# agnusmaximus/Word2Bits

Hardware: AMD Instinct MI355X
Metric: training words/sec at dim=800 bitlevel=1 neg=24 (higher is better)
Workload: dtype f32

## Files before the change

include/word2bits_hip.h:

```cpp
#ifndef WORD2BITS_HIP_H
#define WORD2BITS_HIP_H
#include <stdint.h>
#ifdef __cplusplus
extern "C" {
#endif

#define W2B_OK            0
#define W2B_EINVAL       -1
#define W2B_ENOGPU       -2
#define W2B_EHIP         -3
#define W2B_ENOMEM       -4
#define W2B_EUNSUPPORTED -5
#define W2B_ERCCL        -6
#define W2B_ESTATE       -7
#define W2B_EIO          -8

#define W2B_EXP_TABLE_SIZE 1000
#define W2B_MAX_EXP 6
#define W2B_MAX_SENTENCE_LENGTH 1000
#define W2B_UNIGRAM_TABLE_SIZE 100000000LL

typedef struct w2b_trainer w2b_trainer;

typedef struct w2b_config {
// ... 76 lines not shown
int w2b_export_packed(w2b_trainer *t, uint64_t *out);

int w2b_set_vocab_counts(w2b_trainer *t, const int64_t *cn, int64_t table_size);
int w2b_set_unigram_table(w2b_trainer *t, const int32_t *table, int64_t table_size);
int w2b_set_exp_table(w2b_trainer *t, const float *exp_table);

int w2b_set_corpus(w2b_trainer *t, const int32_t *ids, int64_t n_tokens);
int w2b_set_corpus_device(w2b_trainer *t, const void *ids_dev, int64_t n_tokens);
int w2b_set_corpus_slice(w2b_trainer *t, const int32_t *ids, int64_t n_tokens, int32_t more_follows);
int w2b_set_shards(w2b_trainer *t, const int64_t *starts, const int32_t *first_override );
int w2b_epoch_begin(w2b_trainer *t);
int w2b_train_step(w2b_trainer *t, int64_t max_positions);
int w2b_epoch_status(w2b_trainer *t, int32_t *finished, int64_t *word_count_actual, float *alpha,
                     double *loss_sum);

int w2b_epoch_poll(w2b_trainer *t, int32_t lag, int32_t *finished, int64_t *word_count_actual, float *alpha,
                   double *loss_sum);

int w2b_suggested_threads(w2b_trainer *t, int32_t *out);

int w2b_worker_kernel_info(w2b_trainer *t, int32_t *resident, int32_t *radius, int32_t *column_bytes,
                           int32_t *workgroups_per_cu, int32_t *hot_rows);
int w2b_worker_kernel_lean(w2b_trainer *t, int32_t *lean);

int w2b_train_tuples(w2b_trainer *t, int64_t n, const int32_t *center, const int32_t *ctx_off,
                     const int32_t *ctx, const int32_t *neg, float alpha, int32_t serial,
                     double *loss_out );
int w2b_train_tuples_device(w2b_trainer *t, int64_t n, const void *center_dev, const void *ctx_off_dev,
                            const void *ctx_dev, const void *neg_dev, float alpha, int32_t grid);

int w2b_synchronize(w2b_trainer *t);
int w2b_timing_enable(w2b_trainer *t, int32_t on);
int w2b_timing_read(w2b_trainer *t, double *kernel_ms, int64_t *launches);
int w2b_timing_launches(w2b_trainer *t, double *ms_out, int64_t capacity, int64_t *launches);

#define W2B_UNIQUE_ID_BYTES 128
int w2b_comm_unique_id(void *out128);
int w2b_comm_init(w2b_trainer *t, int32_t nranks, int32_t rank, const void *id128);
int w2b_comm_count(w2b_trainer *t, int32_t *nranks_out);
int w2b_sync_replicas(w2b_trainer *t, int32_t mode);
int64_t w2b_suggested_exchange_words(int64_t train_words_per_epoch, int32_t replicas);
int w2b_sync_stats(w2b_trainer *t, int64_t *exchanges, double *device_ms);

int w2b_exchange_init(w2b_trainer *t);
int w2b_exchange_begin(w2b_trainer *t, int64_t *n_chunks, int64_t *local_word_count );
int w2b_exchange_counts(w2b_trainer *t, void **buf_dev, int64_t *elems);
// ... 61 lines not shown
```

word2bits_amd/_lib.py:

```python
import ctypes as C
import os
import sys

_HERE = os.path.dirname(os.path.abspath(__file__))
LIB_PATH = os.environ.get("W2B_LIB", os.path.join(_HERE, "libword2bits_hip.so"))

W2B_OK, W2B_EINVAL, W2B_ENOGPU, W2B_EHIP, W2B_ENOMEM = 0, -1, -2, -3, -4
W2B_EUNSUPPORTED, W2B_ERCCL, W2B_ESTATE, W2B_EIO = -5, -6, -7, -8
ERROR_NAMES = {-1: "W2B_EINVAL", -2: "W2B_ENOGPU", -3: "W2B_EHIP", -4: "W2B_ENOMEM",
               -5: "W2B_EUNSUPPORTED", -6: "W2B_ERCCL", -7: "W2B_ESTATE", -8: "W2B_EIO"}


class W2bError(RuntimeError):
    def __init__(self, code, text):
        super().__init__("%s (%d): %s" % (ERROR_NAMES.get(code, "?"), code, text))
        self.code = code


class Config(C.Structure):
    _fields_ = [
        ("vocab_size", C.c_int64), ("train_words", C.c_int64), ("iter", C.c_int64),
        ("layer1_size", C.c_int32), ("window", C.c_int32), ("negative", C.c_int32),
        ("bitlevel", C.c_int32), ("num_threads", C.c_int32),
        ("alpha", C.c_float), ("sample", C.c_float), ("reg", C.c_float),
# ... 38 lines not shown
    "w2b_plan_rows": (C.c_int, [C.POINTER(Config), C.POINTER(Tuning), i64p, C.c_int32, C.c_int32, C.POINTER(RowPlan)]),
    "w2b_get_tuning": (C.c_int, [vp, C.POINTER(Tuning)]),
    "w2b_set_tuning": (C.c_int, [vp, C.POINTER(Tuning)]),
    "w2b_init_net": (C.c_int, [vp]),
    "w2b_set_model": (C.c_int, [vp, f32p, f32p]),
    "w2b_get_model": (C.c_int, [vp, f32p, f32p]),
    "w2b_model_device_ptrs": (C.c_int, [vp, C.POINTER(vp), C.POINTER(vp)]),
    "w2b_export_quantized": (C.c_int, [vp, f32p]),
    "w2b_export_packed": (C.c_int, [vp, u64p]),
    "w2b_set_vocab_counts": (C.c_int, [vp, i64p, C.c_int64]),
    "w2b_set_unigram_table": (C.c_int, [vp, i32p, C.c_int64]),
    "w2b_set_exp_table": (C.c_int, [vp, f32p]),
    "w2b_set_corpus": (C.c_int, [vp, i32p, C.c_int64]),
    "w2b_set_corpus_device": (C.c_int, [vp, vp, C.c_int64]),
    "w2b_set_corpus_slice": (C.c_int, [vp, i32p, C.c_int64, C.c_int32]),
    "w2b_set_shards": (C.c_int, [vp, i64p, i32p]),
    "w2b_epoch_begin": (C.c_int, [vp]),
    "w2b_train_step": (C.c_int, [vp, C.c_int64]),
    "w2b_epoch_status": (C.c_int, [vp, i32p, i64p, f32p, f64p]),
    "w2b_epoch_poll": (C.c_int, [vp, C.c_int32, i32p, i64p, f32p, f64p]),
    "w2b_suggested_threads": (C.c_int, [vp, i32p]),
    "w2b_worker_kernel_info": (C.c_int, [vp, i32p, i32p, i32p, i32p, i32p]),
    "w2b_worker_kernel_lean": (C.c_int, [vp, i32p]),
    "w2b_train_tuples": (C.c_int, [vp, C.c_int64, i32p, i32p, i32p, i32p, C.c_float, C.c_int32, f64p]),
    "w2b_train_tuples_device": (C.c_int, [vp, C.c_int64, vp, vp, vp, vp, C.c_float, C.c_int32]),
    "w2b_synchronize": (C.c_int, [vp]),
    "w2b_timing_enable": (C.c_int, [vp, C.c_int32]),
    "w2b_timing_read": (C.c_int, [vp, f64p, i64p]),
    "w2b_timing_launches": (C.c_int, [vp, f64p, C.c_int64, i64p]),
    "w2b_comm_unique_id": (C.c_int, [vp]),
    "w2b_comm_init": (C.c_int, [vp, C.c_int32, C.c_int32, vp]),
    "w2b_comm_count": (C.c_int, [vp, i32p]),
    "w2b_sync_replicas": (C.c_int, [vp, C.c_int32]),
    "w2b_suggested_exchange_words": (C.c_int64, [C.c_int64, C.c_int32]),
    "w2b_sync_stats": (C.c_int, [vp, i64p, f64p]),
    "w2b_exchange_init": (C.c_int, [vp]),
    "w2b_exchange_begin": (C.c_int, [vp, i64p, i64p]),
    "w2b_exchange_counts": (C.c_int, [vp, C.POINTER(vp), i64p]),
    "w2b_exchange_delta": (C.c_int, [vp, C.c_int64, C.POINTER(vp), i64p]),
    "w2b_exchange_apply": (C.c_int, [vp, C.c_int64, C.c_float]),
    "w2b_exchange_end": (C.c_int, [vp, C.c_int64]),
    "w2b_corpus_load": (C.c_int, [C.c_char_p, C.c_int32, C.POINTER(vp)]),
    "w2b_corpus_load_ex": (C.c_int, [C.c_char_p, C.c_int32, C.c_int32, C.POINTER(vp)]),
    "w2b_corpus_free": (None, [vp]),
    "w2b_corpus_vocab_size": (C.c_int64, [vp]),
    "w2b_corpus_train_words": (C.c_int64, [vp]),
# ... 143 lines not shown
```

word2bits_amd/csrc/w2b_device.hpp:

```cpp
#pragma once
#include "w2b_internal.h"
#include <type_traits>

#ifndef W2B_T
#define W2B_T 13
#endif
#ifndef W2B_T_LOSS
#define W2B_T_LOSS W2B_T
#endif
template <bool LOSS> struct TFor { static constexpr int value = LOSS ? W2B_T_LOSS : W2B_T; };
#ifndef W2B_CA
#define W2B_CA 8
#endif
#ifndef W2B_STASH
#define W2B_STASH 8
#endif
#ifndef W2B_MINWAVES
#define W2B_MINWAVES 4
#endif

namespace {

struct QParam { int bitlevel; int steps_i; float steps_f; };

// ... 143 lines not shown
  f32x4_t t;
  t.x = c.e[0]; t.y = c.e[1]; t.z = c.e[2]; t.w = c.e[3];
  *(W2B_LDS f32x4_t *)p = t;
}

#ifdef W2B_PHASE_TIMERS
#define W2B_TICK(k) do { if (timing_) { const unsigned long long n_ = __builtin_readcyclecounter(); \
    atomicAdd(&P.shared->dbg[k], n_ - tick_); tick_ = n_; } } while (0)
#define W2B_COUNT(k) do { if (timing_) atomicAdd(&P.shared->dbg[k], 1ull); } while (0)
#else
#define W2B_TICK(k) do { } while (0)
#define W2B_COUNT(k) do { } while (0)
#endif

struct WordLds {
  int *ctx;
  int *umult;
  int *tgt;
  int *prev;
  int *cend;
  float *red;
  float *stash;
  float *xprod;
};

__device__ __forceinline__ int round4(int x) { return (x + 3) & ~3; }

__device__ __forceinline__ WordLds carve_word_lds(int *base, int window, int negative, int vec) {
  const int maxc = round4(2 * window + 1), maxt = round4(negative + 1);
  WordLds L;
  L.stash = reinterpret_cast<float *>(base);
  base += W2B_STASH * blockDim.x * vec;
  L.red = reinterpret_cast<float *>(base);
  int *p = base + 2 * W2B_T * W2B_MAXW;
  L.ctx = p; p += maxc;
  L.umult = p; p += maxc;
  L.tgt = p; p += maxt;
  L.prev = p; p += maxt;
  L.cend = p; p += maxt;
  L.xprod = nullptr;
  return L;
}


template <int T, typename IP>
__device__ __forceinline__ int prep_lists(IP tgt, IP prev, IP cend, int nt, IP ctx, IP umult, int cw,
                                          int lane) {
  W2B_WAVE_SYNC();
  for (int i0 = 0; i0 < nt; i0 += 64) {
    const int i = i0 + lane;
    const int me = (i < nt) ? tgt[i] : -1;
    int pd = -1;
    for (int j = 0; j < min(nt, i0 + 64); j++) {
      const int tj = (j >= i0) ? __builtin_amdgcn_readlane(me, j - i0) : tgt[j];
      pd = (j < i && tj == me) ? j : pd;
    }
    if (i < nt) prev[i] = pd;
  }
  if (umult) {
    for (int i0 = 0; i0 < cw; i0 += 64) {
      const int i = i0 + lane;
      const int me = (i < cw) ? ctx[i] : -1;
      bool first = true;
// ... 181 lines not shown
                                             double &loss_acc, const XHot &X) {
  static_assert(!LEAN || (VEC == 4 && MM == 0 && ATOM == 0 && TB == 0 && QM <= 2), "lean form: see w2b_workers_lean");
  constexpr bool REG = !LEAN;
  constexpr bool ATOM_U = !(VEC == 4 && ATOM < 1), ATOM_V = !(VEC == 4 && ATOM < 2);
  constexpr bool THIRDS = LEAN && QM == 1;
  constexpr float third = 1.f / 3.f;
  const int tid = threadIdx.x, lane = tid & 63, wave = tid >> 6, nwaves = blockDim.x >> 6;
  const int dim = P.dim, col0 = tid * VEC;
  const bool active = col0 < dim;
  const float ar2 = REG ? (2.f * alpha) * P.reg : 0.f;
  constexpr int TC = TFor<LOSS>::value;

  Col<VEC> x[TC];
  int rows[TC];
  int start = 0, chunk = 0, end = L.cend[0];
  auto chunk_rows = [&]() {
    const int mine = L.tgt[min(start + lane, nt - 1)];
#pragma unroll
    for (int i = 0; i < TC; i++) rows[i] = __builtin_amdgcn_readlane(mine, i);
  };
  chunk_rows();
  const int nhu = (VEC == 4) ? X.nu : 0, nhv = (VEC == 4) ? X.nv : 0;
  [[maybe_unused]] const int rowb = dim * 4, lane_off = active ? col0 * 4 : (int)W2B_NO_LANE;
  [[maybe_unused]] __amdgpu_buffer_rsrc_t res_u, res_v, res_cu, res_cv;
  if constexpr (LEAN) {
    res_u = __builtin_amdgcn_make_buffer_rsrc((void *)P.u, 0, (int)P.tab_bytes, 0x27000);
    res_v = __builtin_amdgcn_make_buffer_rsrc((void *)P.v, 0, (int)P.tab_bytes, 0x27000);
    res_cu = __builtin_amdgcn_make_buffer_rsrc((void *)X.cu, 0, nhu * rowb, 0x27000);
    res_cv = __builtin_amdgcn_make_buffer_rsrc((void *)X.cv, 0, nhv * rowb, 0x27000);
  }
  auto ld_u = [&](int row) -> Col<VEC> {
    if constexpr (VEC == 4) { if ((unsigned)(row - 1) < (unsigned)nhu) return xhot_ld(X.cu, row - 1, nhu, dim, col0); }
    return load_col<VEC, MM, TB>(P.u, row, dim, col0, P.tab_bytes);
  };
  [[maybe_unused]] const int atomic_rank = ATOM_V ? P.atomic_rank : 0, atomic_rank_u = ATOM_U ? P.atomic_rank_u : 0;
  auto up_u = [&](int row, const Col<VEC> &val, const Col<VEC> &d) {
    if constexpr (VEC == 4) { if ((unsigned)(row - 1) < (unsigned)nhu) { xhot_st(X.cu, row - 1, nhu, dim, col0, val); return; } }
    if constexpr (ATOM_U) { if (row <= atomic_rank_u) { add_col<VEC, TB>(P.u, row, dim, col0, d, P.tab_bytes); return; } }
    store_col<VEC, MM, TB>(P.u, row, dim, col0, val, P.tab_bytes);
  };
  auto ld_v = [&](int row) -> Col<VEC> {
    if constexpr (VEC == 4) { if ((unsigned)(row - 1) < (unsigned)nhv) return xhot_ld(X.cv, row - 1, nhv, dim, col0); }
    return load_col<VEC, MM, TB>(P.v, row, dim, col0, P.tab_bytes);
  };
  auto up_v = [&](int row, const Col<VEC> &val, const Col<VEC> &d) {
    if constexpr (VEC == 4) { if ((unsigned)(row - 1) < (unsigned)nhv) { xhot_st(X.cv, row - 1, nhv, dim, col0, val); return; } }
// ... 10 lines not shown
      if (zero) {
#pragma unroll
        for (int e = 0; e < VEC; e++) x[i].e[e] = 0.f;
      }
      if constexpr (LEAN) { if (start + i < end) x[i] = lean_ld_v(rows[i]); }
      else if (active && start + i < end) x[i] = ld_v(rows[i]);
    }
  };
  load_targets(true);

  Col<VEC> avg;
  float regsq = 0.f;
  const bool reg_on = REG && P.reg != 0.f;
  float *fsave = reinterpret_cast<float *>(L.prev);
#pragma unroll
  for (int e = 0; e < VEC; e++) avg.e[e] = 0.f;
  for (int j0 = 0; j0 < cw; j0 += W2B_CA) {
    Col<VEC> r[W2B_CA];
    if constexpr (LEAN) {
      const int mine = L.ctx[min(j0 + lane, cw - 1)];
#pragma unroll
      for (int jj = 0; jj < W2B_CA; jj++)
        if (j0 + jj < cw) r[jj] = lean_ld_u(__builtin_amdgcn_readlane(mine, jj));
    } else {
#pragma unroll
      for (int jj = 0; jj < W2B_CA; jj++)
        if (active && j0 + jj < cw) r[jj] = ld_u(__builtin_amdgcn_readfirstlane(L.ctx[j0 + jj]));
    }
#pragma unroll
    for (int jj = 0; jj < W2B_CA; jj++)
      if ((LEAN || active) && j0 + jj < cw) {
        if (j0 + jj < W2B_STASH) {
#pragma unroll
          for (int e = 0; e < VEC; e++) L.stash[((j0 + jj) * blockDim.x + tid) * VEC + e] = r[jj].e[e];
        }
#pragma unroll
        for (int e = 0; e < VEC; e++) {
          const float q = quant<QM>(r[jj].e[e], qp);
          avg.e[e] += q;
          if (LOSS && reg_on) regsq += q * q;
        }
      }
  }
  {
    const float cwf = (float)cw;
#pragma unroll
    for (int e = 0; e < VEC; e++) avg.e[e] = active ? avg.e[e] / cwf : 0.f;
  }
  [[maybe_unused]] Col<VEC> avg3;
  if constexpr (THIRDS) {
#pragma unroll
    for (int e = 0; e < VEC; e++) avg3.e[e] = avg.e[e] * third;
  }

  Col<VEC> err;
#pragma unroll
  for (int e = 0; e < VEC; e++) err.e[e] = 0.f;
  int par = 0;
  for (;;) {
    const int n = end - start;
    float p[TC];
#pragma unroll
    for (int i = 0; i < TC; i++) {
      float t[VEC];
#pragma unroll
      for (int e = 0; e < VEC; e++) {
        if constexpr (THIRDS) t[e] = (x[i].e[e] < 0.f) ? -avg3.e[e] : avg3.e[e];
        else {
          const float q = quant<QM>(x[i].e[e], qp);
          t[e] = avg.e[e] * q;
        }
      }
      const float s = (VEC == 4) ? (t[0] + t[1 % VEC]) + (t[2 % VEC] + t[3 % VEC]) : ((VEC == 2) ? t[0] + t[1 % VEC] : t[0]);
      p[i] = active ? s : 0.f;
    }
    float *red = L.red + par * (TC * W2B_MAXW);
    if (MM == W2B_MM_EXACT) {
      float fchain = 0.f;
      for (int b0 = 0; b0 < dim; b0 += W2B_EXACT_COLS) {
        if (active && col0 >= b0 && col0 < b0 + W2B_EXACT_COLS) {
#pragma unroll
          for (int i = 0; i < TC; i++)
            if (i < n) {
#pragma unroll
              for (int e = 0; e < VEC; e++)
                L.xprod[i * (W2B_EXACT_COLS + 1) + (col0 - b0) + e] = avg.e[e] * quant<QM>(x[i].e[e], qp);
            }
        }
        __syncthreads();
        if (wave == 0 && lane < n) {
          const int cnt = min(W2B_EXACT_COLS, dim - b0);
          const float *src = L.xprod + lane * (W2B_EXACT_COLS + 1);
          for (int c = 0; c < cnt; c++) fchain += src[c];
        }
        __syncthreads();
      }
      if (wave == 0 && lane < n) {
        red[lane * W2B_MAXW] = fchain;
        for (int w = 1; w < nwaves; w++) red[lane * W2B_MAXW + w] = 0.f;
      }
    } else {
#pragma unroll
      for (int i = 0; i < TC; i++) p[i] = wave_sum(p[i]);
      if (lane == 0) {
#pragma unroll
        for (int i = 0; i < TC; i++)
          if (i < n) red[i * W2B_MAXW + wave] = p[i];
      }
    }
    __syncthreads();
    float gl = 0.f;
    if (lane < n) {
      float f = 0.f;
      for (int w = 0; w < nwaves; w++) f += red[lane * W2B_MAXW + w];
      gl = grad_scalar(f, start + lane == 0, alpha, P.exp_table);
      if (LOSS && wave == 0) fsave[start + lane] = f;
    }
#pragma unroll
    for (int i = 0; i < TC; i++) {
      if (i < n) {
        const float g = __int_as_float(__builtin_amdgcn_readlane(__float_as_int(gl), i));
        [[maybe_unused]] const float g3 = g * third;
        const bool by_add = (VEC == 4 && ATOM >= 2) && rows[i] <= atomic_rank && !((unsigned)(rows[i] - 1) < (unsigned)nhv);
        Col<VEC> dl;
        if constexpr (VEC == 4 && ATOM >= 2) {
#pragma unroll
          for (int e = 0; e < VEC; e++) dl.e[e] = 0.f;
        }
        if constexpr (LEAN) {
#pragma unroll
          for (int h = 0; h < 4; h += 2) {
            f32x2_t xv = {x[i].e[h], x[i].e[h + 1]};
            if (QM != 0) asm volatile("" : "+v"(xv));
            f32x2_t ge;
            if constexpr (THIRDS) { ge.x = (xv.x < 0.f) ? -g3 : g3; ge.y = (xv.y < 0.f) ? -g3 : g3; }
            else { ge.x = quant<QM>(xv.x, qp); ge.y = quant<QM>(xv.y, qp); ge = g * ge; }
            const f32x2_t ev = f32x2_t{err.e[h], err.e[h + 1]} + ge;
            err.e[h] = ev.x; err.e[h + 1] = ev.y;
// ... 21 lines not shown
        }
        if constexpr (VEC == 4 && ATOM >= 2) {
          if (by_add) add_col_contig<TB>(P.v, rows[i], dim, dl, P.tab_bytes);
        }
      }
    }
    start = end;
    if (start >= nt) break;
    end = L.cend[++chunk];
    par ^= 1;
    chunk_rows();
    load_targets(false);
  }

  for (int j0 = 0; j0 < cw; j0 += W2B_CA) {
    Col<VEC> r[W2B_CA];
    if constexpr (LEAN) {
      const int mine = L.ctx[min(j0 + lane, cw - 1)], mult = (j0 + lane < cw) ? L.umult[min(j0 + lane, cw - 1)] : 0;
      const int how_l = (j0 + lane < W2B_STASH && mine > P.fresh_rank_u) ? mult : -mult;
      if (j0 < W2B_STASH) {
        static_assert(W2B_STASH % W2B_CA == 0, "a sub-chunk lies inside the stash or beyond it");
        Col<4> rs[W2B_CA];
#pragma unroll
        for (int jj = 0; jj < W2B_CA; jj++) rs[jj] = lds_ld((const W2B_LDS float *)(L.stash + ((j0 + jj) * blockDim.x + tid) * VEC));
#pragma unroll
        for (int jj = 0; jj < W2B_CA; jj++) {
          const int how = __builtin_amdgcn_readlane(how_l, jj);
          for (int k = 0; k < how; k++) {
#pragma unroll
            for (int e = 0; e < VEC; e++) rs[jj].e[e] = rs[jj].e[e] + err.e[e];
          }
          lean_st(res_u, res_cu, nhu, rowb, __builtin_amdgcn_readlane(mine, jj), how > 0 ? lane_off : (int)W2B_NO_LANE, rs[jj]);
        }
      }
      if (__ballot(lane < W2B_CA && how_l < 0) != 0ull) {
#pragma unroll
        for (int jj = 0; jj < W2B_CA; jj++)
          if (__builtin_amdgcn_readlane(how_l, jj) < 0) r[jj] = lean_ld_u(__builtin_amdgcn_readlane(mine, jj));
        __builtin_amdgcn_s_waitcnt(0x0F70);
#pragma unroll
        for (int jj = 0; jj < W2B_CA; jj++) {
          const int how = __builtin_amdgcn_readlane(how_l, jj);
          if (how < 0) {
            for (int k = 0; k < -how; k++) {
#pragma unroll
              for (int e = 0; e < VEC; e++) r[jj].e[e] = r[jj].e[e] + err.e[e];
            }
// ... 358 lines not shown
```

word2bits_amd/csrc/w2b_internal.h:

```cpp
#pragma once
#include <hip/hip_runtime.h>
#include <stdint.h>

#define W2B_LCG_A 25214903917ULL
#define W2B_LCG_C 11ULL
#define W2B_MAX_SEN 1000
#define W2B_MAXW 16
#define W2B_NXCD 8
#define W2B_XHOT_MAX 128

struct W2bShared {
  float alpha;
  int pad0;
  unsigned long long word_count_actual;
  double loss_tuples;
  int workers_done;
  int corpus_overrun;
  unsigned long long wca_others;
  unsigned long long wca_at_sync;
  double loss_epoch;
  int launch_done, pad1;
  unsigned long long dbg[16];
};

// ... 25 lines not shown
  unsigned long long table_magic, window_magic;
  int dim, window, negative, bitlevel, num_threads;
  int total_threads;
  int mem_mode;
  float *entry;
  float *xhot;
  int xhot_u, xhot_v;
  int hot_period;
  int xhot_m;
  int uavg_rank;
  int win_refresh;
  float xhot_w;
  float *wide_scratch;
  int wide;
  int atomic_rank;
  int atomic_rank_u;
  int fresh_rank_u;
  int exact;
  int rc_rows;
  float *rc;
  int *rc_flags;
  int worker_base;
  float starting_alpha, sample, reg;
};

struct w2b_config;
struct w2b_tuning;
void w2b_shape_params(W2bParams &p, const w2b_config &cfg, const w2b_tuning &tune);

int w2b_block_threads(int dim, int *vec_out, int *wide_out = nullptr);
size_t w2b_lds_bytes(int dim, int window, int negative, bool worker_form, bool exact = false);
int w2b_tuple_max_grid(int num_cus);
hipError_t w2b_launch_tuples(const W2bParams &p, long long n, const int32_t *center,
                             const int32_t *ctx_off, const int32_t *ctx, const int32_t *neg,
                             float alpha, int grid, int num_cus, int per_cu_override, bool loss,
                             hipStream_t s);
hipError_t w2b_launch_workers(const W2bParams &p, long long max_positions, bool loss, hipStream_t s, int grid = 0,
                              bool force_generic = false);
bool w2b_workers_lean(const W2bParams &p, bool force_generic);
int w2b_resident_plan(int dim, int window, int negative);
bool w2b_resident_atomic_ok(const W2bParams &p, int radius);
long long w2b_resident_scratch_rows(int radius);
hipError_t w2b_launch_resident(const W2bParams &p, long long max_positions, int radius, bool loss, hipStream_t s,
                               bool debug = false);
bool w2b_groups_ok(const W2bParams &p);
size_t w2b_groups_lds_bytes(int dim, int window, int negative);
int w2b_groups_per_cu(const W2bParams &p, bool loss);
hipError_t w2b_launch_groups(const W2bParams &p, long long max_positions, bool loss, hipStream_t s);
hipError_t w2b_launch_refresher(const W2bParams &p, hipStream_t s);
#define W2B_RC_MAX 64
#define W2B_RC_BLOCKS 16
int w2b_workers_per_cu(const W2bParams &p, bool loss);
int w2b_resident_per_cu(const W2bParams &p, int radius, bool loss);
hipError_t w2b_launch_init_net(float *u, float *v, long long n_per_table, const float *lut,
                               hipStream_t s);
hipError_t w2b_launch_export(const float *u, const float *v, float *out, long long n, int bitlevel,
                             hipStream_t s);
hipError_t w2b_launch_export_packed(const float *u, const float *v, unsigned long long *out, long long rows, int dim,
                                    int bitlevel, hipStream_t s);
hipError_t w2b_launch_eval_normalize(float *M, long long words, long long size, long long ld, int bitlevel,
                                     int fused, float *len_scratch, hipStream_t s);
hipError_t w2b_launch_eval_queries(const float *M, long long ld, long long nq, const int *b1, const int *b2,
                                   const int *b3, float *Q, int variant, hipStream_t s);
hipError_t w2b_launch_eval_scores(const float *Q, const float *M, int nq, int words, int size, int ld, int fused,
                                  const int *b1, const int *b2, const int *b3, unsigned long long *best,
                                  int variant , hipStream_t s);
void w2b_eval_topk_layout(long long words, int k, bool mfma, int *nunits, int *cap);
hipError_t w2b_launch_eval_topk(const float *Q, const float *M, int nq, int words, int size, int ld, int fused,
                                const int *b1, const int *b2, const int *b3, int k, unsigned long long *bound,
                                unsigned long long *bkt, unsigned long long *keys, unsigned char *cnt,
                                unsigned long long *out, int variant, hipStream_t s);
hipError_t w2b_launch_bits_planes(const uint32_t *B, int nw, int dim, int nq, long long nqp, const int *b1, const int *b2,
                                  const int *b3, uint32_t *P, hipStream_t s);
void w2b_bits_layout(long long words, long long nq, int topk, int max_splits, int *splits, int *rows_per_split);
hipError_t w2b_launch_bits_top1(const uint32_t *B, int words, int dim, const uint32_t *P, long long nqp, int nq,
// ... 129 lines not shown
```

word2bits_amd/csrc/w2b_kernels_misc.hip:

```cpp
#include "w2b_device.hpp"

namespace {
__global__ void k_init_net(float *u, float *v, long long n, const float *__restrict__ lut) {
  const long long stride = (long long)gridDim.x * blockDim.x;
  for (long long i = (long long)blockIdx.x * blockDim.x + threadIdx.x; i < n; i += stride) {
    v[i] = lut[i & 65535];
    u[i] = lut[(n + i) & 65535];
  }
}

template <int QM>
__global__ void k_export(const float *__restrict__ u, const float *__restrict__ v, float *__restrict__ out,
                         long long n, QParam qp) {
  typedef float f4 __attribute__((ext_vector_type(4)));
  const long long stride = (long long)gridDim.x * blockDim.x;
  const bool aligned = ((((size_t)u) | ((size_t)v) | ((size_t)out)) & 15) == 0;
  const long long n4 = aligned ? (n >> 2) : 0;
  for (long long i = (long long)blockIdx.x * blockDim.x + threadIdx.x; i < n4; i += stride) {
    const f4 a = reinterpret_cast<const f4 *>(u)[i], b = reinterpret_cast<const f4 *>(v)[i];
    f4 o;
    o.x = quant<QM>(a.x + b.x, qp); o.y = quant<QM>(a.y + b.y, qp);
    o.z = quant<QM>(a.z + b.z, qp); o.w = quant<QM>(a.w + b.w, qp);
    reinterpret_cast<f4 *>(out)[i] = o;
  }
// ... 147 lines not shown
__global__ void k_wca_pack(const W2bShared *sh, unsigned long long *buf) { buf[0] = sh->word_count_actual; }
__global__ void k_wca_unpack(W2bShared *sh, const unsigned long long *buf) {
  sh->wca_others = buf[1] - buf[0];
  sh->wca_at_sync = buf[0];
}

}

int w2b_block_threads(int dim, int *vec_out, int *wide_out) {
  int vec = (dim % 4 == 0) ? 4 : 1;
  const int cols = dim / vec;
  int threads = ((cols + 63) / 64) * 64;
  int wide = 0;
  if (threads > 1024) {
    threads = 1024;
    vec = 1;
    wide = 1;
  }
  if (vec_out) *vec_out = vec;
  if (wide_out) *wide_out = wide;
  return threads;
}

size_t w2b_lds_bytes(int dim, int window, int negative, bool worker_form, bool exact) {
  const int maxc = (2 * window + 1 + 3) & ~3, maxt = (negative + 1 + 3) & ~3;
  int vec;
  const int threads = w2b_block_threads(dim, &vec);
  size_t ints = (size_t)W2B_STASH * threads * vec + 2 * W2B_T * W2B_MAXW + 2 * maxc + 3 * maxt;
  if (worker_form) ints += ((W2B_MAX_SEN + 3) & ~3) + 4 + (sizeof(WorkerLds) + 3) / 4 + 4;
  else ints += 4;
  if (exact) ints += (size_t)W2B_T * (W2B_EXACT_COLS + 1) + 4;
  return ints * 4;
}

hipError_t w2b_launch_init_net(float *u, float *v, long long n, const float *lut, hipStream_t s) {
  hipLaunchKernelGGL(k_init_net, dim3(2048), dim3(256), 0, s, u, v, n, lut);
  return hipGetLastError();
}

hipError_t w2b_launch_export(const float *u, const float *v, float *out, long long n, int bitlevel,
                             hipStream_t s) {
  QParam qp;
  qp.bitlevel = bitlevel;
  qp.steps_i = (bitlevel >= 4) ? (1 << (bitlevel - 1)) : 1;
  qp.steps_f = (float)qp.steps_i;
  return dispatch_q(bitlevel, [&](auto qm) -> hipError_t {
    constexpr int QM = decltype(qm)::value;
    hipLaunchKernelGGL((k_export<QM>), dim3(2048), dim3(256), 0, s, u, v, out, n, qp);
    return hipGetLastError();
  });
}
// ... 52 lines not shown
```

word2bits_amd/csrc/w2b_kernels_workers.hip:

```cpp
#include "w2b_device.hpp"

namespace {

template <int QM, int VEC, bool LOSS, int MAXTHREADS, int MM, int ATOM = 0, int TB = -1, bool LEAN = false>
__global__ void __launch_bounds__(MAXTHREADS, (MAXTHREADS <= 256 ? W2B_MINWAVES : 1)) k_train_workers(const W2bParams P, const long long max_positions) {
  extern __shared__ int smem[];
  WordLds L = carve_word_lds(smem, P.window, P.negative, VEC);
  int *s_sen = L.cend + round4(P.negative + 1);
  WorkerLds *S = reinterpret_cast<WorkerLds *>(s_sen + round4(W2B_MAX_SEN) + 4);
  if (MM == W2B_MM_EXACT) L.xprod = reinterpret_cast<float *>(reinterpret_cast<int *>(S) + (sizeof(WorkerLds) + 3) / 4 + 4);
  const int tid = threadIdx.x, lane = tid & 63, wave = tid >> 6;
  const int wid = blockIdx.x + P.worker_base;
  if (wid >= P.num_threads) return;
  W2bWorker *G = P.workers + wid;
  if (G->done) return;
  const QParam qp = make_qparam(P);
  copy_sentence(s_sen, G->sen, G->sen_len, tid, blockDim.x);
  if (tid == 0) worker_restore(G, S);
  __syncthreads();
  double loss_acc = 0.0;
  const bool hot = (VEC == 4 && MM == 0 && P.xhot != nullptr && P.xhot_u + P.xhot_v > 0);
  XHot XH = xhot_here(P);
  if (!hot) { XH.nu = 0; XH.nv = 0; }
  int since_merge = 0, merge_cursor = (wid >> 3) * P.xhot_m;
  const int W = P.window;
  for (long long it = 0; it < max_positions; ++it) {
    if (wave == 0) {
      unsigned long long rng = S->rng;
      long long cursor = S->cursor, wc = S->wc, last_wc = S->last_wc;
      int sen_len = S->sen_len, sen_pos = S->sen_pos, ovr = S->override_, eof = S->eof;
      int done = 0, cw = 0, nt = 0;
      float alpha = 0.f;
      alpha_schedule_step(P, wc, last_wc, lane);
      if (sen_len == 0) {
        read_sentence(P, s_sen, rng, cursor, wc, ovr, eof, sen_len, lane);
        sen_pos = 0;
        W2B_WAVE_SYNC();
      }
      if (eof || wc > P.train_words / P.total_threads) {
        epoch_end(P, wc, last_wc, lane);
        done = 1;
// ... 33 lines not shown
      if (wide) { if constexpr (VEC == 1 && MAXTHREADS == 1024) process_word_wide<QM, LOSS, MM>(P, L, qp, cw, nt, alpha, loss_acc); }
      else process_word<QM, VEC, LOSS, MM, ATOM, TB, LEAN>(P, L, qp, cw, nt, alpha, loss_acc, XH);
    } else __syncthreads();
    if (VEC == 4 && hot && ++since_merge >= P.hot_period) {
      since_merge = 0;
      xhot_merge_event<MM, TB>(P, XH, merge_cursor, tid * VEC, tid * VEC < P.dim);
    }
  }
  __syncthreads();
  copy_sentence(G->sen, s_sen, S->sen_len, tid, blockDim.x);
  double lsum = 0.0;
  if (LOSS) {
    if (wave == 0) lsum = wave_sum_d(loss_acc);
    else if (lane == 0 && loss_acc != 0.0) { atomicAdd(&G->loss, loss_acc); atomicAdd(&P.shared->loss_epoch, loss_acc); }
  }
  if (tid == 0) {
    if (LOSS) { atomicAdd(&G->loss, lsum); atomicAdd(&P.shared->loss_epoch, lsum); }
    worker_save(P, G, S);
  }
}

}

int w2b_workers_per_cu(const W2bParams &p, bool loss) {
  int vec;
  const int threads = w2b_block_threads(p.dim, &vec);
  const size_t lds = w2b_lds_bytes(p.dim, p.window, p.negative, true, p.exact != 0);
  int nb = 0;
  (void)dispatch_mm_exact(p.mem_mode, p.exact, [&](auto mm) -> hipError_t {
    constexpr int MM = decltype(mm)::value;
    return dispatch_q(p.bitlevel, [&](auto qm) -> hipError_t {
      constexpr int QM = decltype(qm)::value;
      if (threads <= 256) return hipOccupancyMaxActiveBlocksPerMultiprocessor(&nb, k_train_workers<QM, 4, false, 256, MM>, threads, lds);
      return hipOccupancyMaxActiveBlocksPerMultiprocessor(&nb, k_train_workers<QM, 4, false, 1024, MM>, threads, lds);
    });
  });
  return nb > 0 ? nb : 1;
}

bool w2b_workers_lean(const W2bParams &p, bool force_generic) {
  int vec;
  const int threads = w2b_block_threads(p.dim, &vec);
  return !force_generic && vec == 4 && threads <= 256 && p.mem_mode == 0 && !p.exact && p.tab_bytes != 0 && p.atomic_rank <= 0 &&
         p.atomic_rank_u <= 0 && p.reg == 0.f && p.bitlevel >= 0 && p.bitlevel <= 2;
}

hipError_t w2b_launch_workers(const W2bParams &p, long long max_positions, bool loss, hipStream_t s, int grid, bool force_generic) {
  if (grid <= 0) grid = p.num_threads - p.worker_base;
  int vec;
  const int threads = w2b_block_threads(p.dim, &vec);
  const size_t lds = w2b_lds_bytes(p.dim, p.window, p.negative, true, p.exact != 0);
  return dispatch_mm_exact(p.mem_mode, p.exact, [&](auto mm) -> hipError_t {
  constexpr int MM = decltype(mm)::value;
  return dispatch_q(p.bitlevel, [&](auto qm) -> hipError_t {
    constexpr int QM = decltype(qm)::value;
#define W2B_LAUNCH_W(VEC, LOSS) \
    do { if (threads <= 256) hipLaunchKernelGGL((k_train_workers<QM, VEC, LOSS, 256, MM>), dim3(grid), dim3(threads), lds, s, p, max_positions); \
         else hipLaunchKernelGGL((k_train_workers<QM, VEC, LOSS, 1024, MM>), dim3(grid), dim3(threads), lds, s, p, max_positions); } while (0)
    if constexpr (MM == 0) {
      const int atom = p.atomic_rank > 0 ? 2 : (p.atomic_rank_u > 0 ? 1 : 0);
      if constexpr (QM <= 2) {
        if (w2b_workers_lean(p, force_generic)) {
          if (loss) hipLaunchKernelGGL((k_train_workers<QM, 4, true, 256, 0, 0, 0, true>), dim3(grid), dim3(threads), lds, s, p, max_positions);
          else hipLaunchKernelGGL((k_train_workers<QM, 4, false, 256, 0, 0, 0, true>), dim3(grid), dim3(threads), lds, s, p, max_positions);
          return hipGetLastError();
        }
      }
      if (vec == 4 && threads <= 256 && (atom || p.tab_bytes != 0)) {
#define W2B_LAUNCH_A(LOSS, ATOM, TB) hipLaunchKernelGGL((k_train_workers<QM, 4, LOSS, 256, 0, ATOM, TB>), dim3(grid), dim3(threads), lds, s, p, max_positions)
#define W2B_LAUNCH_AT(LOSS, ATOM) do { if (p.tab_bytes != 0) W2B_LAUNCH_A(LOSS, ATOM, 0); else W2B_LAUNCH_A(LOSS, ATOM, -1); } while (0)
        if (atom == 2) { if (loss) W2B_LAUNCH_AT(true, 2); else W2B_LAUNCH_AT(false, 2); }
        else if (atom == 1) { if (loss) W2B_LAUNCH_AT(true, 1); else W2B_LAUNCH_AT(false, 1); }
        else { if (loss) W2B_LAUNCH_A(true, 0, 0); else W2B_LAUNCH_A(false, 0, 0); }
#undef W2B_LAUNCH_AT
// ... 13 lines not shown
```

word2bits_amd/csrc/w2b_trainer.cpp:

```cpp
#include "../../include/word2bits_corpus.h"
#include "w2b_exchange.h"
#include "w2b_host.h"

#include <cmath>
#include <cstdio>
#include <cstdlib>
#include <cstring>

static thread_local std::string g_err;
int w2b_internal_fail(int code, const char *msg) { g_err = msg ? msg : ""; return code; }

extern "C" const char *w2b_version(void) { return "word2bits-hip 0.1 (gfx950)"; }
extern "C" const char *w2b_last_error(void) { return g_err.c_str(); }

extern "C" int w2b_device_count(void) {
  int n = 0;
  if (hipGetDeviceCount(&n) != hipSuccess) return 0;
  return n;
}

extern "C" int w2b_device_compute_units(int32_t device) {
  int n = 0;
  if (hipGetDeviceCount(&n) != hipSuccess || device < 0 || device >= n) return 0;
  hipDeviceProp_t prop;
// ... 520 lines not shown
  if (nu + nv == 0) return W2B_OK;
  const size_t need = (size_t)W2B_NXCD * ((size_t)2 * (nu + nv) * t->in.cfg.layer1_size + (size_t)(nu + nv) * W2B_MAXW);
  bool fresh = (nu != t->xhot_nu || nv != t->xhot_nv);
  if (int rc = grow(t, t->xhot, need, &fresh)) return rc;
  p.xhot = t->xhot;
  if (fresh) {
    HIPCHK(hipMemsetAsync(t->xhot, 0, sizeof(float) * need, t->stream));
    t->xhot_nu = nu;
    t->xhot_nv = nv;
    t->xhot_master_changed = true;
  }
  if (t->xhot_master_changed) HIPCHK(w2b_launch_xhot_fold(p, t->stream));
  t->xhot_master_changed = false;
  return W2B_OK;
}

extern "C" int w2b_suggested_threads(w2b_trainer *t, int32_t *out) {
  NEED(t);
  if (!out) return fail(W2B_EINVAL, "w2b_suggested_threads: null");
  const W2bLaunchPlan lp = w2b_plan_launch(t->in, w2b_plan_probe_workers(t->in));
  W2bParams p{};
  w2b_shape_params(p, t->in.cfg, t->in.tune);
  const int per_cu = lp.radius >= 0 ? w2b_resident_per_cu(p, lp.radius, t->in.cfg.compute_loss != 0)
                                    : w2b_workers_per_cu(p, t->in.cfg.compute_loss != 0);
  *out = (int32_t)w2b_plan_suggested_workers(t->in, lp, (long long)per_cu * t->in.num_cus);
  return W2B_OK;
}

extern "C" int w2b_worker_kernel_info(w2b_trainer *t, int32_t *resident, int32_t *radius, int32_t *column_bytes,
                                      int32_t *workgroups_per_cu, int32_t *hot_rows) {
  NEED(t);
  const W2bLaunchPlan lp = w2b_plan_launch(t->in, t->in.cfg.num_threads);
  W2bParams p{};
  w2b_shape_params(p, t->in.cfg, t->in.tune);
  const bool loss = t->in.cfg.compute_loss != 0;
  if (resident) *resident = lp.kernel;
  if (radius) *radius = lp.radius;
  if (hot_rows) *hot_rows = lp.copies_v;
  int vec = 0;
  (void)w2b_block_threads(t->in.cfg.layer1_size, &vec);
  if (column_bytes) *column_bytes = 4 * (lp.radius >= 0 ? 4 : vec);
  if (workgroups_per_cu)
    *workgroups_per_cu = lp.kernel == W2B_KERNEL_RESIDENT ? w2b_resident_per_cu(p, lp.radius, loss)
                                                          : (lp.kernel == W2B_KERNEL_GROUPS ? w2b_groups_per_cu(p, loss) : w2b_workers_per_cu(p, loss));
  return W2B_OK;
}

extern "C" int w2b_worker_kernel_lean(w2b_trainer *t, int32_t *lean) {
  NEED(t);
  if (!lean) return fail(W2B_EINVAL, "w2b_worker_kernel_lean: null");
  const W2bLaunchPlan lp = w2b_plan_launch(t->in, t->in.cfg.num_threads);
  const W2bParams p = make_params(t, lp);
  *lean = (lp.kernel == W2B_KERNEL_PLAIN && w2b_workers_lean(p, t->generic_worker)) ? 1 : 0;
  return W2B_OK;
}

extern "C" int w2b_train_step(w2b_trainer *t, int64_t max_positions) {
  NEED(t);
  if (!t->corpus || !t->shards_set) return fail(W2B_ESTATE, "w2b_train_step: corpus/shards not set");
  if (max_positions <= 0) return fail(W2B_EINVAL, "w2b_train_step: max_positions must be positive");
  const W2bLaunchPlan lp = w2b_plan_launch(t->in, t->in.cfg.num_threads);
  if (lp.kernel == W2B_KERNEL_RESIDENT)
    if (int rc = grow(t, t->entry,
                      (size_t)t->in.cfg.num_threads * (size_t)w2b_resident_scratch_rows(lp.radius) * t->in.cfg.layer1_size)) return rc;
  W2bParams p = make_params(t, lp);
  if (int rc = xhot_prepare(t, p)) return rc;
  if (int rc = wide_prepare(t, p, t->in.cfg.num_threads)) return rc;

  w2b_xchg_add_words(t->xchg, (long long)max_positions * t->in.cfg.num_threads);
  HIPCHK(timing_begin(t));
  if (lp.kernel == W2B_KERNEL_RESIDENT) HIPCHK(w2b_launch_resident(p, max_positions, lp.radius, t->in.cfg.compute_loss != 0, t->stream, t->debug));
  else if (lp.kernel == W2B_KERNEL_GROUPS) {
    if (int rc = rc_prepare(t, p, lp)) return rc;
    if (p.rc_rows > 0) HIPCHK(hipEventRecord(t->rc_go, t->stream));
    HIPCHK(w2b_launch_groups(p, max_positions, t->in.cfg.compute_loss != 0, t->stream));
    if (p.rc_rows > 0) {
// ... 149 lines not shown
```

word2bits_amd/trainer.py:

```python
import ctypes as C
import numpy as np

from . import _lib
from ._lib import Config, check, lib


def _f32(a):
    return a.ctypes.data_as(_lib.f32p)


def _i32(a):
    return a.ctypes.data_as(_lib.i32p)


def _i64(a):
    return a.ctypes.data_as(_lib.i64p)


def packed_words_per_row(dim, bitlevel):
    n = lib().w2b_packed_words_per_row(int(dim), int(bitlevel))
    if n < 0:
        raise _lib.W2bError(_lib.W2B_EUNSUPPORTED, "bit-packed vectors exist for bitlevel 1 and 2")
    return n

# ... 207 lines not shown
        return bool(fin.value), wca.value, alpha.value, loss.value

    def train_epoch(self, positions_per_launch=4096):
        self.epoch_begin()
        while True:
            self.train_step(positions_per_launch)
            fin, _, _, loss = self.epoch_status()
            if fin:
                return loss

    def worker_kernel_info(self):
        a, b, c, d, e = C.c_int32(0), C.c_int32(0), C.c_int32(0), C.c_int32(0), C.c_int32(0)
        check(lib().w2b_worker_kernel_info(self._h, C.byref(a), C.byref(b), C.byref(c), C.byref(d), C.byref(e)))
        return a.value == 1, b.value, c.value, d.value, e.value

    def worker_kernel_name(self):
        a = C.c_int32(0)
        check(lib().w2b_worker_kernel_info(self._h, C.byref(a), None, None, None, None))
        return ("plain", "resident", "groups")[a.value]

    def worker_kernel_lean(self):
        a = C.c_int32(0)
        check(lib().w2b_worker_kernel_lean(self._h, C.byref(a)))
        return a.value == 1

    def suggested_threads(self):
        n = C.c_int32(0)
        check(lib().w2b_suggested_threads(self._h, C.byref(n)))
        return n.value

    def train_tuples(self, center, ctx_off, ctx, neg, alpha, serial=False):
        center = np.ascontiguousarray(center, np.int32)
        ctx_off = np.ascontiguousarray(ctx_off, np.int32)
        ctx = np.ascontiguousarray(ctx, np.int32)
        neg = np.ascontiguousarray(neg, np.int32)
        loss = C.c_double(0)
        check(lib().w2b_train_tuples(self._h, len(center), _i32(center), _i32(ctx_off), _i32(ctx), _i32(neg),
                                     float(alpha), int(bool(serial)), C.byref(loss)))
        return loss.value

    def train_tuples_device(self, n, center_ptr, ctx_off_ptr, ctx_ptr, neg_ptr, alpha, grid=0):
        check(lib().w2b_train_tuples_device(self._h, int(n), _lib.vp(center_ptr), _lib.vp(ctx_off_ptr),
                                            _lib.vp(ctx_ptr), _lib.vp(neg_ptr), float(alpha), int(grid)))

    def synchronize(self):
        check(lib().w2b_synchronize(self._h))
# ... 114 lines not shown
```

Baseline: 30.64 million.

## Shrink lean worker LDS layout and stage exp table in LDS

For the lean worker kernel, the stash is now sized by dim columns instead of threads*vec, and stash rows are written by the lean load path. The reduction buffer uses a 4-wide stride so each target's partials are read as one f32x4. The exp table is copied into LDS when doing so does not lower occupancy, so sigmoid lookups avoid global memory. This adds per-launch table copy cost and extra LDS, and changes the stash indexing.

```diff
diff --git a/include/word2bits_hip.h b/include/word2bits_hip.h
--- a/include/word2bits_hip.h
+++ b/include/word2bits_hip.h
@@ -122,6 +122,7 @@
 int w2b_worker_kernel_info(w2b_trainer *t, int32_t *resident, int32_t *radius, int32_t *column_bytes,
                            int32_t *workgroups_per_cu, int32_t *hot_rows);
 int w2b_worker_kernel_lean(w2b_trainer *t, int32_t *lean);
+int w2b_worker_kernel_table_lds(w2b_trainer *t, int32_t *in_lds);
 
 int w2b_train_tuples(w2b_trainer *t, int64_t n, const int32_t *center, const int32_t *ctx_off,
                      const int32_t *ctx, const int32_t *neg, float alpha, int32_t serial,
diff --git a/word2bits_amd/_lib.py b/word2bits_amd/_lib.py
--- a/word2bits_amd/_lib.py
+++ b/word2bits_amd/_lib.py
@@ -84,6 +84,7 @@
     "w2b_suggested_threads": (C.c_int, [vp, i32p]),
     "w2b_worker_kernel_info": (C.c_int, [vp, i32p, i32p, i32p, i32p, i32p]),
     "w2b_worker_kernel_lean": (C.c_int, [vp, i32p]),
+    "w2b_worker_kernel_table_lds": (C.c_int, [vp, i32p]),
     "w2b_train_tuples": (C.c_int, [vp, C.c_int64, i32p, i32p, i32p, i32p, C.c_float, C.c_int32, f64p]),
     "w2b_train_tuples_device": (C.c_int, [vp, C.c_int64, vp, vp, vp, vp, C.c_float, C.c_int32]),
     "w2b_synchronize": (C.c_int, [vp]),
diff --git a/word2bits_amd/csrc/w2b_device.hpp b/word2bits_amd/csrc/w2b_device.hpp
--- a/word2bits_amd/csrc/w2b_device.hpp
+++ b/word2bits_amd/csrc/w2b_device.hpp
@@ -189,23 +189,27 @@
   float *red;
   float *stash;
   float *xprod;
+  float *etab;
 };
+#define W2B_LEAN_MAXW 4
 
 __device__ __forceinline__ int round4(int x) { return (x + 3) & ~3; }
 
-__device__ __forceinline__ WordLds carve_word_lds(int *base, int window, int negative, int vec) {
+__device__ __forceinline__ WordLds carve_word_lds(int *base, int window, int negative, int vec, int stash_ints = 0,
+                                                  int red_w = W2B_MAXW) {
   const int maxc = round4(2 * window + 1), maxt = round4(negative + 1);
   WordLds L;
   L.stash = reinterpret_cast<float *>(base);
-  base += W2B_STASH * blockDim.x * vec;
+  base += W2B_STASH * (stash_ints ? stash_ints : blockDim.x * vec);
   L.red = reinterpret_cast<float *>(base);
-  int *p = base + 2 * W2B_T * W2B_MAXW;
+  int *p = base + 2 * W2B_T * red_w;
   L.ctx = p; p += maxc;
   L.umult = p; p += maxc;
   L.tgt = p; p += maxt;
   L.prev = p; p += maxt;
   L.cend = p; p += maxt;
   L.xprod = nullptr;
+  L.etab = nullptr;
   return L;
 }
 
@@ -433,6 +437,8 @@
   chunk_rows();
   const int nhu = (VEC == 4) ? X.nu : 0, nhv = (VEC == 4) ? X.nv : 0;
   [[maybe_unused]] const int rowb = dim * 4, lane_off = active ? col0 * 4 : (int)W2B_NO_LANE;
+  [[maybe_unused]] const int scols = (dim + 3) >> 2;
+  constexpr int RW = LEAN ? W2B_LEAN_MAXW : W2B_MAXW;
   [[maybe_unused]] __amdgpu_buffer_rsrc_t res_u, res_v, res_cu, res_cv;
   if constexpr (LEAN) {
     res_u = __builtin_amdgcn_make_buffer_rsrc((void *)P.u, 0, (int)P.tab_bytes, 0x27000);
@@ -489,6 +495,11 @@
 #pragma unroll
       for (int jj = 0; jj < W2B_CA; jj++)
         if (j0 + jj < cw) r[jj] = lean_ld_u(__builtin_amdgcn_readlane(mine, jj));
+      if (j0 < W2B_STASH && active) {
+#pragma unroll
+        for (int jj = 0; jj < W2B_CA; jj++)
+          if (j0 + jj < cw) lds_st((W2B_LDS float *)(L.stash + ((j0 + jj) * scols + tid) * 4), r[jj]);
+      }
     } else {
 #pragma unroll
       for (int jj = 0; jj < W2B_CA; jj++)
@@ -497,7 +508,7 @@
 #pragma unroll
     for (int jj = 0; jj < W2B_CA; jj++)
       if ((LEAN || active) && j0 + jj < cw) {
-        if (j0 + jj < W2B_STASH) {
+        if (!LEAN && j0 + jj < W2B_STASH) {
 #pragma unroll
           for (int e = 0; e < VEC; e++) L.stash[((j0 + jj) * blockDim.x + tid) * VEC + e] = r[jj].e[e];
         }
@@ -541,7 +552,7 @@
       const float s = (VEC == 4) ? (t[0] + t[1 % VEC]) + (t[2 % VEC] + t[3 % VEC]) : ((VEC == 2) ? t[0] + t[1 % VEC] : t[0]);
       p[i] = active ? s : 0.f;
     }
-    float *red = L.red + par * (TC * W2B_MAXW);
+    float *red = L.red + par * (TC * RW);
     if (MM == W2B_MM_EXACT) {
       float fchain = 0.f;
       for (int b0 = 0; b0 < dim; b0 += W2B_EXACT_COLS) {
@@ -563,8 +574,8 @@
         __syncthreads();
       }
       if (wave == 0 && lane < n) {
-        red[lane * W2B_MAXW] = fchain;
-        for (int w = 1; w < nwaves; w++) red[lane * W2B_MAXW + w] = 0.f;
+        red[lane * RW] = fchain;
+        for (int w = 1; w < nwaves; w++) red[lane * RW + w] = 0.f;
       }
     } else {
 #pragma unroll
@@ -572,15 +583,26 @@
       if (lane == 0) {
 #pragma unroll
         for (int i = 0; i < TC; i++)
-          if (i < n) red[i * W2B_MAXW + wave] = p[i];
+          if (i < n) red[i * RW + wave] = p[i];
       }
     }
     __syncthreads();
     float gl = 0.f;
     if (lane < n) {
       float f = 0.f;
-      for (int w = 0; w < nwaves; w++) f += red[lane * W2B_MAXW + w];
-      gl = grad_scalar(f, start + lane == 0, alpha, P.exp_table);
+      if constexpr (LEAN) {
+        static_assert(W2B_LEAN_MAXW == 4, "one f32x4 per target");
+        const f32x4_t r4 = *(const W2B_LDS f32x4_t *)(red + lane * RW);
+        f += r4.x;
+        f += (nwaves > 1) ? r4.y : 0.f;
+        f += (nwaves > 2) ? r4.z : 0.f;
+        f += (nwaves > 3) ? r4.w : 0.f;
+        if (L.etab) gl = grad_scalar(f, start + lane == 0, alpha, (const W2B_LDS float *)L.etab);
+        else gl = grad_scalar(f, start + lane == 0, alpha, P.exp_table);
+      } else {
+        for (int w = 0; w < nwaves; w++) f += red[lane * W2B_MAXW + w];
+        gl = grad_scalar(f, start + lane == 0, alpha, P.exp_table);
+      }
       if (LOSS && wave == 0) fsave[start + lane] = f;
     }
 #pragma unroll
@@ -648,7 +670,7 @@
         static_assert(W2B_STASH % W2B_CA == 0, "a sub-chunk lies inside the stash or beyond it");
         Col<4> rs[W2B_CA];
 #pragma unroll
-        for (int jj = 0; jj < W2B_CA; jj++) rs[jj] = lds_ld((const W2B_LDS float *)(L.stash + ((j0 + jj) * blockDim.x + tid) * VEC));
+        for (int jj = 0; jj < W2B_CA; jj++) rs[jj] = lds_ld((const W2B_LDS float *)(L.stash + ((j0 + jj) * scols + tid) * 4));
 #pragma unroll
         for (int jj = 0; jj < W2B_CA; jj++) {
           const int how = __builtin_amdgcn_readlane(how_l, jj);
diff --git a/word2bits_amd/csrc/w2b_internal.h b/word2bits_amd/csrc/w2b_internal.h
--- a/word2bits_amd/csrc/w2b_internal.h
+++ b/word2bits_amd/csrc/w2b_internal.h
@@ -71,6 +71,7 @@
   int *rc_flags;
   int worker_base;
   float starting_alpha, sample, reg;
+  int exp_lds;
 };
 
 struct w2b_config;
@@ -78,7 +79,8 @@
 void w2b_shape_params(W2bParams &p, const w2b_config &cfg, const w2b_tuning &tune);
 
 int w2b_block_threads(int dim, int *vec_out, int *wide_out = nullptr);
-size_t w2b_lds_bytes(int dim, int window, int negative, bool worker_form, bool exact = false);
+size_t w2b_lds_bytes(int dim, int window, int negative, bool worker_form, bool exact = false, bool lean = false);
+#define W2B_EXP_LDS_BYTES 4000
 int w2b_tuple_max_grid(int num_cus);
 hipError_t w2b_launch_tuples(const W2bParams &p, long long n, const int32_t *center,
                              const int32_t *ctx_off, const int32_t *ctx, const int32_t *neg,
@@ -87,6 +89,7 @@
 hipError_t w2b_launch_workers(const W2bParams &p, long long max_positions, bool loss, hipStream_t s, int grid = 0,
                               bool force_generic = false);
 bool w2b_workers_lean(const W2bParams &p, bool force_generic);
+size_t w2b_workers_carve(const W2bParams &p, bool loss, bool force_generic, int *exp_lds);
 int w2b_resident_plan(int dim, int window, int negative);
 bool w2b_resident_atomic_ok(const W2bParams &p, int radius);
 long long w2b_resident_scratch_rows(int radius);
@@ -99,7 +102,7 @@
 hipError_t w2b_launch_refresher(const W2bParams &p, hipStream_t s);
 #define W2B_RC_MAX 64
 #define W2B_RC_BLOCKS 16
-int w2b_workers_per_cu(const W2bParams &p, bool loss);
+int w2b_workers_per_cu(const W2bParams &p, bool loss, bool force_generic = false);
 int w2b_resident_per_cu(const W2bParams &p, int radius, bool loss);
 hipError_t w2b_launch_init_net(float *u, float *v, long long n_per_table, const float *lut,
                                hipStream_t s);
diff --git a/word2bits_amd/csrc/w2b_kernels_misc.hip b/word2bits_amd/csrc/w2b_kernels_misc.hip
--- a/word2bits_amd/csrc/w2b_kernels_misc.hip
+++ b/word2bits_amd/csrc/w2b_kernels_misc.hip
@@ -193,11 +193,13 @@
   return threads;
 }
 
-size_t w2b_lds_bytes(int dim, int window, int negative, bool worker_form, bool exact) {
+size_t w2b_lds_bytes(int dim, int window, int negative, bool worker_form, bool exact, bool lean) {
   const int maxc = (2 * window + 1 + 3) & ~3, maxt = (negative + 1 + 3) & ~3;
   int vec;
   const int threads = w2b_block_threads(dim, &vec);
-  size_t ints = (size_t)W2B_STASH * threads * vec + 2 * W2B_T * W2B_MAXW + 2 * maxc + 3 * maxt;
+  size_t ints = lean ? (size_t)W2B_STASH * ((dim + 3) / 4) * 4 + 2 * W2B_T * W2B_LEAN_MAXW
+                     : (size_t)W2B_STASH * threads * vec + 2 * W2B_T * W2B_MAXW;
+  ints += 2 * maxc + 3 * maxt;
   if (worker_form) ints += ((W2B_MAX_SEN + 3) & ~3) + 4 + (sizeof(WorkerLds) + 3) / 4 + 4;
   else ints += 4;
   if (exact) ints += (size_t)W2B_T * (W2B_EXACT_COLS + 1) + 4;
diff --git a/word2bits_amd/csrc/w2b_kernels_workers.hip b/word2bits_amd/csrc/w2b_kernels_workers.hip
--- a/word2bits_amd/csrc/w2b_kernels_workers.hip
+++ b/word2bits_amd/csrc/w2b_kernels_workers.hip
@@ -5,10 +5,12 @@
 template <int QM, int VEC, bool LOSS, int MAXTHREADS, int MM, int ATOM = 0, int TB = -1, bool LEAN = false>
 __global__ void __launch_bounds__(MAXTHREADS, (MAXTHREADS <= 256 ? W2B_MINWAVES : 1)) k_train_workers(const W2bParams P, const long long max_positions) {
   extern __shared__ int smem[];
-  WordLds L = carve_word_lds(smem, P.window, P.negative, VEC);
+  WordLds L = LEAN ? carve_word_lds(smem, P.window, P.negative, VEC, ((P.dim + 3) >> 2) * 4, W2B_LEAN_MAXW)
+                   : carve_word_lds(smem, P.window, P.negative, VEC);
   int *s_sen = L.cend + round4(P.negative + 1);
   WorkerLds *S = reinterpret_cast<WorkerLds *>(s_sen + round4(W2B_MAX_SEN) + 4);
-  if (MM == W2B_MM_EXACT) L.xprod = reinterpret_cast<float *>(reinterpret_cast<int *>(S) + (sizeof(WorkerLds) + 3) / 4 + 4);
+  float *const tail = reinterpret_cast<float *>(reinterpret_cast<int *>(S) + (sizeof(WorkerLds) + 3) / 4 + 4);
+  if (MM == W2B_MM_EXACT) L.xprod = tail;
   const int tid = threadIdx.x, lane = tid & 63, wave = tid >> 6;
   const int wid = blockIdx.x + P.worker_base;
   if (wid >= P.num_threads) return;
@@ -17,6 +19,12 @@
   const QParam qp = make_qparam(P);
   copy_sentence(s_sen, G->sen, G->sen_len, tid, blockDim.x);
   if (tid == 0) worker_restore(G, S);
+  if constexpr (LEAN) {
+    if (P.exp_lds) {
+      for (int i = tid; i < W2B_EXP_LDS_BYTES / 4; i += blockDim.x) tail[i] = P.exp_table[i];
+      L.etab = tail;
+    }
+  }
   __syncthreads();
   double loss_acc = 0.0;
   const bool hot = (VEC == 4 && MM == 0 && P.xhot != nullptr && P.xhot_u + P.xhot_v > 0);
@@ -96,11 +104,47 @@
 
 }
 
-int w2b_workers_per_cu(const W2bParams &p, bool loss) {
+bool w2b_workers_lean(const W2bParams &p, bool force_generic) {
   int vec;
   const int threads = w2b_block_threads(p.dim, &vec);
-  const size_t lds = w2b_lds_bytes(p.dim, p.window, p.negative, true, p.exact != 0);
+  return !force_generic && vec == 4 && threads <= 256 && p.mem_mode == 0 && !p.exact && p.tab_bytes != 0 && p.atomic_rank <= 0 &&
+         p.atomic_rank_u <= 0 && p.reg == 0.f && p.bitlevel >= 0 && p.bitlevel <= 2;
+}
+
+static int lean_occupancy(const W2bParams &p, bool loss, int threads, size_t lds) {
   int nb = 0;
+  (void)dispatch_q(p.bitlevel, [&](auto qm) -> hipError_t {
+    constexpr int QM = decltype(qm)::value;
+    if constexpr (QM <= 2) {
+      if (loss) return hipOccupancyMaxActiveBlocksPerMultiprocessor(&nb, k_train_workers<QM, 4, true, 256, 0, 0, 0, true>, threads, lds);
+      return hipOccupancyMaxActiveBlocksPerMultiprocessor(&nb, k_train_workers<QM, 4, false, 256, 0, 0, 0, true>, threads, lds);
+    }
+    return hipSuccess;
+  });
+  return nb;
+}
+
+size_t w2b_workers_carve(const W2bParams &p, bool loss, bool force_generic, int *exp_lds) {
+  if (exp_lds) *exp_lds = 0;
+  if (!w2b_workers_lean(p, force_generic)) return w2b_lds_bytes(p.dim, p.window, p.negative, true, p.exact != 0);
+  const size_t lds = w2b_lds_bytes(p.dim, p.window, p.negative, true, false, true);
+  int vec;
+  const int threads = w2b_block_threads(p.dim, &vec);
+  const int without = lean_occupancy(p, loss, threads, lds);
+  if (without > 0 && lean_occupancy(p, loss, threads, lds + W2B_EXP_LDS_BYTES) >= without) {
+    if (exp_lds) *exp_lds = 1;
+    return lds + W2B_EXP_LDS_BYTES;
+  }
+  return lds;
+}
+
+int w2b_workers_per_cu(const W2bParams &p, bool loss, bool force_generic) {
+  int vec;
+  const int threads = w2b_block_threads(p.dim, &vec);
+  const size_t lds = w2b_workers_carve(p, loss, force_generic, nullptr);
+  int nb = 0;
+  if (w2b_workers_lean(p, force_generic)) nb = lean_occupancy(p, loss, threads, lds);
+  else
   (void)dispatch_mm_exact(p.mem_mode, p.exact, [&](auto mm) -> hipError_t {
     constexpr int MM = decltype(mm)::value;
     return dispatch_q(p.bitlevel, [&](auto qm) -> hipError_t {
@@ -112,18 +156,12 @@
   return nb > 0 ? nb : 1;
 }
 
-bool w2b_workers_lean(const W2bParams &p, bool force_generic) {
+hipError_t w2b_launch_workers(const W2bParams &p_in, long long max_positions, bool loss, hipStream_t s, int grid, bool force_generic) {
+  if (grid <= 0) grid = p_in.num_threads - p_in.worker_base;
   int vec;
-  const int threads = w2b_block_threads(p.dim, &vec);
-  return !force_generic && vec == 4 && threads <= 256 && p.mem_mode == 0 && !p.exact && p.tab_bytes != 0 && p.atomic_rank <= 0 &&
-         p.atomic_rank_u <= 0 && p.reg == 0.f && p.bitlevel >= 0 && p.bitlevel <= 2;
-}
-
-hipError_t w2b_launch_workers(const W2bParams &p, long long max_positions, bool loss, hipStream_t s, int grid, bool force_generic) {
-  if (grid <= 0) grid = p.num_threads - p.worker_base;
-  int vec;
-  const int threads = w2b_block_threads(p.dim, &vec);
-  const size_t lds = w2b_lds_bytes(p.dim, p.window, p.negative, true, p.exact != 0);
+  const int threads = w2b_block_threads(p_in.dim, &vec);
+  W2bParams p = p_in;
+  const size_t lds = w2b_workers_carve(p, loss, force_generic, &p.exp_lds);
   return dispatch_mm_exact(p.mem_mode, p.exact, [&](auto mm) -> hipError_t {
   constexpr int MM = decltype(mm)::value;
   return dispatch_q(p.bitlevel, [&](auto qm) -> hipError_t {
diff --git a/word2bits_amd/csrc/w2b_trainer.cpp b/word2bits_amd/csrc/w2b_trainer.cpp
--- a/word2bits_amd/csrc/w2b_trainer.cpp
+++ b/word2bits_amd/csrc/w2b_trainer.cpp
@@ -566,7 +566,7 @@
   W2bParams p{};
   w2b_shape_params(p, t->in.cfg, t->in.tune);
   const int per_cu = lp.radius >= 0 ? w2b_resident_per_cu(p, lp.radius, t->in.cfg.compute_loss != 0)
-                                    : w2b_workers_per_cu(p, t->in.cfg.compute_loss != 0);
+                                    : w2b_workers_per_cu(p, t->in.cfg.compute_loss != 0, t->generic_worker);
   *out = (int32_t)w2b_plan_suggested_workers(t->in, lp, (long long)per_cu * t->in.num_cus);
   return W2B_OK;
 }
@@ -586,7 +586,7 @@
   if (column_bytes) *column_bytes = 4 * (lp.radius >= 0 ? 4 : vec);
   if (workgroups_per_cu)
     *workgroups_per_cu = lp.kernel == W2B_KERNEL_RESIDENT ? w2b_resident_per_cu(p, lp.radius, loss)
-                                                          : (lp.kernel == W2B_KERNEL_GROUPS ? w2b_groups_per_cu(p, loss) : w2b_workers_per_cu(p, loss));
+                                                          : (lp.kernel == W2B_KERNEL_GROUPS ? w2b_groups_per_cu(p, loss) : w2b_workers_per_cu(p, loss, t->generic_worker));
   return W2B_OK;
 }
 
@@ -596,6 +596,17 @@
   const W2bLaunchPlan lp = w2b_plan_launch(t->in, t->in.cfg.num_threads);
   const W2bParams p = make_params(t, lp);
   *lean = (lp.kernel == W2B_KERNEL_PLAIN && w2b_workers_lean(p, t->generic_worker)) ? 1 : 0;
+  return W2B_OK;
+}
+
+extern "C" int w2b_worker_kernel_table_lds(w2b_trainer *t, int32_t *in_lds) {
+  NEED(t);
+  if (!in_lds) return fail(W2B_EINVAL, "w2b_worker_kernel_table_lds: null");
+  const W2bLaunchPlan lp = w2b_plan_launch(t->in, t->in.cfg.num_threads);
+  const W2bParams p = make_params(t, lp);
+  int e = 0;
+  if (lp.kernel == W2B_KERNEL_PLAIN) (void)w2b_workers_carve(p, t->in.cfg.compute_loss != 0, t->generic_worker, &e);
+  *in_lds = e;
   return W2B_OK;
 }
 
diff --git a/word2bits_amd/trainer.py b/word2bits_amd/trainer.py
--- a/word2bits_amd/trainer.py
+++ b/word2bits_amd/trainer.py
@@ -253,6 +253,11 @@
     def worker_kernel_lean(self):
         a = C.c_int32(0)
         check(lib().w2b_worker_kernel_lean(self._h, C.byref(a)))
+        return a.value == 1
+
+    def worker_kernel_table_lds(self):
+        a = C.c_int32(0)
+        check(lib().w2b_worker_kernel_table_lds(self._h, C.byref(a)))
         return a.value == 1
 
     def suggested_threads(self):
```

After: 30.77 million (median of 3 runs). About the same (+0.4%).
